# lasgroup/Model-based-policy-optimizers

Hardware: AMD Instinct MI355X
Metric: model-rollout transitions/sec + SAC updates/sec, Pendulum 5-ens h=5 (higher is better)
Workload: dtype f32

## Files before the change

### include/mbpo_hip.h

```cpp
#ifndef MBPO_HIP_H
#define MBPO_HIP_H

#include <stdint.h>

#ifdef __cplusplus
extern "C" {
#endif

#define MBPO_OK 0
#define MBPO_ERR_ARG (-1)
#define MBPO_ERR_UNSUPPORTED (-2)
#define MBPO_ERR_LAUNCH (-3)

#define MBPO_MAX_LAYERS 8

#define MBPO_ACT_SWISH 0
#define MBPO_ACT_RELU 1
#define MBPO_ACT_TANH 2

typedef struct mbpo_mlp_desc {
  const float *params;
  int64_t net_stride;
  int32_t n_nets;
  int32_t n_layers;
// ... 118 lines not shown
int mbpo_replay_sample_mixed(const float *data, int64_t max_size, int32_t row_len, const int32_t *state, const float *real_data,
                             int64_t real_max_size, int32_t real_row_len, const int32_t *real_state, uint64_t seed, uint64_t offset,
                             uint64_t real_offset, const uint64_t *rng_dev, int64_t n, int32_t minibatch, int32_t n_real,
                             int32_t *idx_out, float *out, void *stream);

int mbpo_philox_permutation(uint64_t seed, uint64_t offset, const uint64_t *rng_dev, int64_t n, int32_t *perm,
                            uint32_t *workspace, void *stream);

int64_t mbpo_running_stats_workspace_floats(int32_t x_dim);
int mbpo_running_stats_reduce(const float *rows, int64_t n_rows, int32_t row_len, int32_t col_off, int32_t x_dim,
                              const float *stats, float *sums, float *workspace, int32_t pass, void *stream);
int mbpo_running_stats_apply(float *stats, const float *sums, int32_t x_dim, float std_min, float std_max, void *stream);
int mbpo_running_stats_update(const float *rows, int64_t n_rows, int32_t row_len, int32_t col_off, int32_t x_dim, float *stats,
                              float *sums, float *workspace, float std_min, float std_max, void *stream);

int mbpo_gae_scan(const float *truncation, const float *termination, const float *rewards, const float *values,
                  const float *bootstrap, float *vs, float *advantages, int64_t B, int32_t T, float gamma,
                  float lam, int32_t time_major, void *stream);
int mbpo_lambda_return_scan(const float *rewards, const float *next_values, float *returns, int64_t B, int32_t T,
                            float gamma, float lam, int32_t time_major, void *stream);
int mbpo_gae_scan_discounts(const float *truncation, const float *termination, const float *rewards, const float *values,
                            const float *bootstrap, const float *discounts, float *vs, float *advantages, int64_t B,
                            int32_t T, float lam, int32_t time_major, void *stream);

typedef struct mbpo_sac_desc {
  int32_t x_dim, u_dim;
  int32_t policy_layers;
  int32_t policy_dims[MBPO_MAX_LAYERS + 1];
  int32_t q_layers;
  int32_t q_dims[MBPO_MAX_LAYERS + 1];
// ... 209 lines not shown
```

### model-based-policy-optimizers_amd/csrc/knobs.hpp

```cpp
#pragma once

#define MBPO_KNOB_TABLE(X)                                                                                                          \
  X(SAC_LEAN, "MBPO_SAC_LEAN", 1, false, "0: the generic k_sac_fwd_bwd also where k_sac_lean applies")                             \
  X(SAC_LAYERED, "MBPO_SAC_LAYERED", 0, false, "1: force SAC's layer-by-layer path (tests)")                                        \
  X(SAC_SPLIT, "MBPO_SAC_SPLIT", -1, false, "0/1: two / three workgroups per SAC tile; -1: by network shape")                       \
  X(SAC_JVP, "MBPO_SAC_JVP", -1, false, "0: no forward-mode dQ/da in SAC's actor role; -1: where the shapes allow it")              \
        \
  X(SAC_THIN, "MBPO_SAC_THIN", 1, true, "0: SAC's thin first / last layers go through the MFMA runners too")                        \
  X(PPO_LEAN, "MBPO_PPO_LEAN", 1, false, "0: the generic PPO kernels also where k_ppo_lean / k_ppo_vg_lean apply")                  \
  X(PPO_LAYERED, "MBPO_PPO_LAYERED", 0, false, "1: force PPO's layer-by-layer path (tests)")                                        \
  X(PPO_SP2, "MBPO_PPO_SP2", -1, false, "0: never the 512-thread two-per-CU k_ppo_fwd_bwd; -1: by shape and tile count")            \
  X(PPO_VALUES_GAE, "MBPO_PPO_VALUES_GAE", -1, false, "0: separate values / GAE / moments launches; -1: fused where it fits")       \
  X(ENS_LEAN, "MBPO_ENS_LEAN", 1, false, "0: the generic k_ensemble_forward also where k_ens_fwd_lean applies")                     \
  X(ROLLOUT_LEAN, "MBPO_ROLLOUT_LEAN", 1, false, "0 generic 64-wide rollout kernel, 1 k_rollout_lean, 2 / 3 lean with two tiles in flight forced on / off") \
  X(ROLLOUT_PIPE, "MBPO_ROLLOUT_PIPE", -1, false, "0/1: two tiles in flight per k_rollout_lean workgroup off / on; -1: by tile count") \
  X(LAYERED_T2_MIN, "MBPO_LAYERED_T2_MIN", 4096, false, "64x64-tile count from which the layered GEMM keeps 64x64 tiles (below: 32x32)") \
  X(LAYERED_GROUP, "MBPO_LAYERED_GROUP", 1, false, "0: every layered GEMM its own launch instead of one per dependency level")      \
  X(PERM_BUCKETS, "MBPO_PERM_BUCKETS", 1, false, "0: philox_permutation without the bucket pre-sort")                               \
  X(BPTT_ZSTORE_MAX_MB, "MBPO_BPTT_ZSTORE_MAX_MB", 16384, false, "largest BPTT member pre-activation store; above it the backward sweep recomputes") \
  X(ICEM_UPDATE, nullptr, -1, false, "override only: 0 the global-memory k_icem_update, 1 k_icem_update_lds where it fits")         \
  X(BPTT_ZSTORE, nullptr, -1, false, "override only: 0 no BPTT pre-activation store (recompute)")

enum KnobId {
#define MBPO_KNOB_ID_(id, env, dflt, reread, meaning) KNOB_##id,
  MBPO_KNOB_TABLE(MBPO_KNOB_ID_)
#undef MBPO_KNOB_ID_
  KNOB_COUNT
};

long long mbpo_knob(KnobId id);
int mbpo_knob_override(KnobId id);
int mbpo_knob_set_override(KnobId id, int mode);
```

### model-based-policy-optimizers_amd/csrc/replay.hip

```cpp
#include "common.hpp"
#include <stdlib.h>

struct ReplayPos {
  int pos, roll, head;
};

__device__ __forceinline__ ReplayPos replay_plan(const int *state, long long max_size, long long n) {
  ReplayPos p;
  long long pos = state[0];
  long long roll = max_size - pos - n;
  if (roll > 0) roll = 0;
  p.roll = (int)roll;
  p.pos = (int)(pos + roll);
  p.head = (int)(((long long)state[2] - roll) % max_size);
  return p;
}

__global__ void __launch_bounds__(256) k_replay_insert(float *data, long long max_size, int D, const int *state,
                                                        const float *rows, long long n_rows) {
  const ReplayPos p = replay_plan(state, max_size, n_rows);
  const long long s0 = ((long long)p.pos + p.head) % max_size;
  const long long n1 = (max_size - s0) < n_rows ? (max_size - s0) : n_rows;
  const long long e1 = n1 * D, total = n_rows * D;
  float *dst1 = data + s0 * D;
  const long long gtid = (long long)blockIdx.x * blockDim.x + threadIdx.x, gsz = (long long)gridDim.x * blockDim.x;
  const bool vec = ((e1 | total) & 3) == 0 && ((((unsigned long long)dst1) | ((unsigned long long)data) | ((unsigned long long)rows)) & 15ull) == 0;
  if (vec) {
    const f32x4 *src = reinterpret_cast<const f32x4 *>(rows);
    f32x4 *d1 = reinterpret_cast<f32x4 *>(dst1), *d2 = reinterpret_cast<f32x4 *>(data);
    const long long q1 = e1 >> 2, qt = total >> 2;
    for (long long i = gtid; i < qt; i += gsz) {
      const f32x4 v = src[i];
      if (i < q1) d1[i] = v;
      else d2[i - q1] = v;
    }
  } else {
    for (long long i = gtid; i < total; i += gsz) {
      const float v = rows[i];
      if (i < e1) dst1[i] = v;
      else data[i - e1] = v;
    }
  }
}

__global__ void k_replay_advance(int *state, long long max_size, long long n_rows) {
  if (threadIdx.x == 0 && blockIdx.x == 0) {
    const ReplayPos p = replay_plan(state, max_size, n_rows);
    long long newpos = ((long long)p.pos + n_rows) % (max_size + 1);
    long long sp = (long long)state[1] + p.roll;
    state[0] = (int)newpos;
    state[1] = (int)(sp > 0 ? sp : 0);
    state[2] = p.head;
    state[3] = (int)((unsigned)state[3] + (unsigned)n_rows);
  }
}

extern "C" int mbpo_replay_insert(float *data, int64_t max_size, int32_t row_len, int32_t *state, const float *rows,
                                  int64_t n_rows, void *stream) {
  MBPO_REQUIRE(data && state, MBPO_ERR_ARG, "replay_insert: null pointer");
  MBPO_REQUIRE(max_size > 0 && max_size < (1LL << 31) - 1 && row_len > 0, MBPO_ERR_ARG, "replay_insert: bad max_size/row_len");
  MBPO_REQUIRE(n_rows >= 0 && n_rows <= max_size, MBPO_ERR_ARG,
               "replay_insert: %lld rows do not fit a buffer of %lld rows", (long long)n_rows, (long long)max_size);
  if (n_rows == 0) return MBPO_OK;
  MBPO_REQUIRE(rows, MBPO_ERR_ARG, "replay_insert: null rows");
  long long total = n_rows * row_len;
  int grid = (int)((total + 255) / 256 < 2048 ? (total + 255) / 256 : 2048);
  hipStream_t st = (hipStream_t)stream;
  hipLaunchKernelGGL(k_replay_insert, dim3(grid), dim3(256), 0, st, data, (long long)max_size, row_len, state, rows,
                     (long long)n_rows);
  hipLaunchKernelGGL(k_replay_advance, dim3(1), dim3(64), 0, st, state, (long long)max_size, (long long)n_rows);
  MBPO_CHECK_LAUNCH("replay_insert");
  return MBPO_OK;
}

static int gather_rows_per_block(int row_len) {
  const int pieces = (row_len & 3) == 0 ? row_len >> 2 : row_len;
  int rb = (2048 + pieces - 1) / pieces;
  return rb < 1 ? 1 : (rb > 256 ? 256 : rb);
}

template <bool SAMPLE>
__global__ void __launch_bounds__(256) k_replay_gather(const float *data, long long max_size, int D, const int *state,
                                                        const int *idx, unsigned long long seed, unsigned long long offset,
                                                        const unsigned long long *rng_dev, long long n, int *idx_out, float *out, int RB) {
  __shared__ long long s_phys[256];
  if (SAMPLE) {
    const RngKey rk = rng_resolve(seed, offset, rng_dev);
    seed = rk.seed;
    offset = rk.offset;
  }
  const int head = state[2];
  const int lo = state[1], hi = state[0];
  const int tid = threadIdx.x;
  const bool vec = (D & 3) == 0 && ((((unsigned long long)data) | ((unsigned long long)out)) & 15ull) == 0;
  for (long long row0 = (long long)blockIdx.x * RB; row0 < n; row0 += (long long)gridDim.x * RB) {
    const long long j = row0 + tid;
    if (tid < RB && j < n) {
      long long li;
      if (SAMPLE) {
        li = philox_randint(seed, offset, MBPO_STREAM_REPLAY, (unsigned long long)j, lo, hi);
        if (idx_out) idx_out[j] = (int)li;
      } else {
        li = idx[j];
      }
      long long w = li % max_size;
      if (w < 0) w += max_size;
      s_phys[tid] = (w + head) % max_size;
    }
    __syncthreads();
    const int rows_here = (int)((n - row0) < RB ? (n - row0) : RB);
// ... 3 lines not shown
      f32x4 *dst = reinterpret_cast<f32x4 *>(out) + row0 * D4;
      for (int e = tid; e < total; e += 256) {
        const int r = e / D4, c = e - r * D4;
        dst[e] = src[s_phys[r] * D4 + c];
      }
    } else {
      const int total = rows_here * D;
      float *dst = out + row0 * D;
      for (int e = tid; e < total; e += 256) {
        const int r = e / D, c = e - r * D;
        dst[e] = data[s_phys[r] * D + c];
      }
    }
    __syncthreads();
  }
}

extern "C" int mbpo_replay_gather(const float *data, int64_t max_size, int32_t row_len, const int32_t *state,
                                  const int32_t *idx, int64_t n, float *out, void *stream) {
  MBPO_REQUIRE(data && state, MBPO_ERR_ARG, "replay_gather: null pointer");
  MBPO_REQUIRE(max_size > 0 && row_len > 0 && n >= 0, MBPO_ERR_ARG, "replay_gather: bad sizes");
  if (n == 0) return MBPO_OK;
  MBPO_REQUIRE(idx && out, MBPO_ERR_ARG, "replay_gather: null idx/out");
  const int RB = gather_rows_per_block(row_len);
  int grid = (int)((n + RB - 1) / RB < 4096 ? (n + RB - 1) / RB : 4096);
  hipLaunchKernelGGL(k_replay_gather<false>, dim3(grid), dim3(256), 0, (hipStream_t)stream, data, (long long)max_size, row_len,
                     state, idx, 0ull, 0ull, (const unsigned long long *)nullptr, (long long)n, (int *)nullptr, out, RB);
  MBPO_CHECK_LAUNCH("replay_gather");
  return MBPO_OK;
}
// ... 99 lines not shown
                     (unsigned long long)offset, (unsigned long long)real_offset, (const unsigned long long *)rng_dev, (long long)n,
                     minibatch, n_real, idx_out, out, RB);
  MBPO_CHECK_LAUNCH("replay_sample_mixed");
  return MBPO_OK;
}

#define STATS_WGS 512

__device__ __forceinline__ float wave_sum(float v) {
#pragma unroll
  for (int o = 32; o > 0; o >>= 1) v += __shfl_down(v, o, 64);
  return v;
}

template <int PASS>
__global__ void __launch_bounds__(256) k_stats_partial(const float *rows, long long n_rows, int D, int col_off, int X,
                                                        const float *stats, const float *sums, float *partial) {
  const int tid = threadIdx.x;
  const float *mean = stats + 1;
  const int rows_per_pass = 256 / X;
  const int c = tid % X, r0 = tid / X;
  float acc = 0.f;
  if (r0 < rows_per_pass) {
    const float m = mean[c];
    float upd = 0.f;
    if (PASS == 1) upd = sums[1 + c] / (stats[0] + sums[0]);
    for (long long r = (long long)blockIdx.x * rows_per_pass + r0; r < n_rows; r += (long long)gridDim.x * rows_per_pass) {
      float d = rows[r * D + col_off + c] - m;
      acc += (PASS == 0) ? d : d * (d - upd);
    }
  }
  __shared__ float s_all[256];
  s_all[tid] = acc;
  __syncthreads();
  if (tid < X) {
    float a = 0.f;
    for (int t = tid; t < rows_per_pass * X; t += X) a += s_all[t];
    partial[(long long)blockIdx.x * X + tid] = a;
  }
}

__device__ __forceinline__ float stats_column_sums(const float *partial, int n_parts, int X, float *s_sl) {
  const int tid = threadIdx.x;
  const int nsl = 256 / X, c = tid % X, sl = tid / X;
  float acc = 0.f;
  if (sl < nsl) {
    int g = sl;
    for (; g + 7 * nsl < n_parts; g += 8 * nsl) {
      float v[8];
#pragma unroll
      for (int k = 0; k < 8; ++k) v[k] = partial[(long long)(g + k * nsl) * X + c];
#pragma unroll
      for (int k = 0; k < 8; ++k) acc += v[k];
    }
// ... 57 lines not shown
    float s = sqrtf(fmaxf(nsv, 0.f) / count);
    sd[c] = fminf(fmaxf(s, std_min), std_max);
  }
  __syncthreads();
  if (c == 0) stats[0] = count;
}

extern "C" int mbpo_running_stats_apply(float *stats, const float *sums, int32_t x_dim, float std_min, float std_max, void *stream) {
  MBPO_REQUIRE(stats && sums, MBPO_ERR_ARG, "running_stats_apply: null pointer");
  MBPO_REQUIRE(x_dim > 0 && x_dim <= 128, MBPO_ERR_ARG, "running_stats_apply: x_dim out of range");
  hipLaunchKernelGGL(k_stats_apply, dim3(1), dim3(128), 0, (hipStream_t)stream, stats, sums, x_dim, std_min, std_max);
  MBPO_CHECK_LAUNCH("running_stats_apply");
  return MBPO_OK;
}

__global__ void __launch_bounds__(256) k_stats_pass1_fused(const float *rows, long long n_rows, int D, int col_off, int X,
                                                           const float *stats, const float *partial0, int n_parts0, float *sums,
                                                           float *partial1) {
  __shared__ float s_all[256];
  __shared__ float s_sum0[128];
  const int tid = threadIdx.x;
  const float tot = stats_column_sums(partial0, n_parts0, X, s_all);
  if (tid < X) {
    s_sum0[tid] = tot;
    if (blockIdx.x == 0) sums[1 + tid] = tot;
  }
  if (blockIdx.x == 0 && tid == 0) sums[0] = (float)n_rows;
  __syncthreads();
  const float *mean = stats + 1;
  const int rows_per_pass = 256 / X;
  const int c = tid % X, r0 = tid / X;
  float acc = 0.f;
  if (r0 < rows_per_pass) {
    const float m = mean[c];
    const float upd = s_sum0[c] / (stats[0] + (float)n_rows);
    for (long long r = (long long)blockIdx.x * rows_per_pass + r0; r < n_rows; r += (long long)gridDim.x * rows_per_pass) {
      float d = rows[r * D + col_off + c] - m;
      acc += d * (d - upd);
    }
  }
  s_all[tid] = acc;
  __syncthreads();
  if (tid < X) {
    float a = 0.f;
    for (int t = tid; t < rows_per_pass * X; t += X) a += s_all[t];
    partial1[(long long)blockIdx.x * X + tid] = a;
  }
}

__global__ void __launch_bounds__(256) k_stats_sums1_apply(const float *partial1, int n_parts, int X, float *sums, float *stats,
                                                           float std_min, float std_max) {
  __shared__ float s_sl[256];
  const int c = threadIdx.x;
  const float a = stats_column_sums(partial1, n_parts, X, s_sl);
  const float count = stats[0] + sums[0];
  if (c < X) {
    sums[1 + X + c] = a;
    if (count > 0.f) {
      float *mean = stats + 1, *sv = stats + 1 + X, *sd = stats + 1 + 2 * X;
      mean[c] = mean[c] + sums[1 + c] / count;
      float nsv = sv[c] + a;
      sv[c] = nsv;
      float s = sqrtf(fmaxf(nsv, 0.f) / count);
      sd[c] = fminf(fmaxf(s, std_min), std_max);
    }
  }
  __syncthreads();
  if (c == 0) stats[0] = count;
}

extern "C" int mbpo_running_stats_update(const float *rows, int64_t n_rows, int32_t row_len, int32_t col_off, int32_t x_dim,
                                         float *stats, float *sums, float *workspace, float std_min, float std_max, void *stream) {
  MBPO_REQUIRE(stats && sums && workspace, MBPO_ERR_ARG, "running_stats_update: null pointer");
  MBPO_REQUIRE(x_dim > 0 && x_dim <= 128 && row_len > 0 && col_off >= 0 && col_off + x_dim <= row_len, MBPO_ERR_ARG,
               "running_stats_update: bad column range (x_dim must be <= 128)");
  MBPO_REQUIRE(n_rows >= 0 && (n_rows == 0 || rows), MBPO_ERR_ARG, "running_stats_update: bad rows");
  hipStream_t st = (hipStream_t)stream;
  int rows_per_pass = 256 / x_dim;
  long long want = (n_rows + rows_per_pass - 1) / rows_per_pass;
  int grid = (int)(want < 1 ? 1 : (want < STATS_WGS ? want : STATS_WGS));
  float *partial1 = workspace + (long long)STATS_WGS * x_dim;
  hipLaunchKernelGGL(k_stats_partial<0>, dim3(grid), dim3(256), 0, st, rows, (long long)n_rows, row_len, col_off, x_dim,
                     (const float *)stats, (const float *)sums, workspace);
  hipLaunchKernelGGL(k_stats_pass1_fused, dim3(grid), dim3(256), 0, st, rows, (long long)n_rows, row_len, col_off, x_dim,
                     (const float *)stats, (const float *)workspace, grid, sums, partial1);
  hipLaunchKernelGGL(k_stats_sums1_apply, dim3(1), dim3(256), 0, st, (const float *)partial1, grid, x_dim, sums, stats, std_min, std_max);
  MBPO_CHECK_LAUNCH("running_stats_update");
  return MBPO_OK;
}

__global__ void __launch_bounds__(256) k_perm_keys(unsigned long long seed, unsigned long long offset, const unsigned long long *rng_dev,
                                                    long long n, unsigned int *keys) {
  const RngKey rk = rng_resolve(seed, offset, rng_dev);
  const long long i = (long long)blockIdx.x * 256 + threadIdx.x;
  if (i >= n) return;
  Philox4 p = philox4x32_10((uint32_t)i, (uint32_t)((unsigned long long)i >> 32), MBPO_STREAM_PERM ^ (uint32_t)(rk.offset >> 32) * 0x9E3779B9u,
                            (uint32_t)rk.offset, (uint32_t)rk.seed, (uint32_t)(rk.seed >> 32));
  keys[i] = p.v[0];
}

__global__ void __launch_bounds__(256) k_perm_rank(const unsigned int *keys, long long n, int *perm) {
  __shared__ unsigned int s_k[1024];
// ... 140 lines not shown
```

### model-based-policy-optimizers_amd/mbpo/_hip.py

```python
from __future__ import annotations

import ctypes as C
import os
from pathlib import Path
from typing import Optional, Sequence

import torch

MBPO_MAX_LAYERS = 8
ACT_IDS = {"swish": 0, "silu": 0, "relu": 1, "tanh": 2}

SYS_PENDULUM, SYS_ENSEMBLE = 0, 1
SYS_GENERIC = 100
ENS_MEAN, ENS_TS1, ENS_TSINF = 0, 1, 2
STREAM_POLICY_NOISE, STREAM_MODEL_NOISE, STREAM_MEMBER = 1, 2, 3
REWARD_PENDULUM, REWARD_QUADRATIC, REWARD_LEARNED = 0, 1, 2

_LIB_PATH = Path(__file__).resolve().parent / "_lib" / "libmbpo_hip.so"


class P2pDesc(C.Structure):
    _fields_ = [("world", C.c_int32), ("rank", C.c_int32), ("n_max", C.c_int64), ("regions", C.c_void_p * 16)]


# ... 178 lines not shown
    _bind_optional(lib)
    _lib = lib
    return lib


def _bind_optional(lib: C.CDLL) -> None:
    i32, i64, u64, f32, vp = C.c_int32, C.c_int64, C.c_uint64, C.c_float, C.c_void_p
    sigs = {
        "mbpo_replay_insert": [vp, i64, i32, vp, vp, i64, vp],
        "mbpo_replay_gather": [vp, i64, i32, vp, vp, i64, vp, vp],
        "mbpo_replay_sample": [vp, i64, i32, vp, u64, u64, vp, i64, vp, vp, vp],
        "mbpo_replay_sample_mixed": [vp, i64, i32, vp, vp, i64, i32, vp, u64, u64, u64, vp, i64, i32, i32, vp, vp, vp],
        "mbpo_running_stats_reduce": [vp, i64, i32, i32, i32, vp, vp, vp, i32, vp],
        "mbpo_running_stats_apply": [vp, vp, i32, f32, f32, vp],
        "mbpo_running_stats_update": [vp, i64, i32, i32, i32, vp, vp, vp, f32, f32, vp],
        "mbpo_gae_scan": [vp, vp, vp, vp, vp, vp, vp, i64, i32, f32, f32, i32, vp],
        "mbpo_gae_scan_discounts": [vp, vp, vp, vp, vp, vp, vp, vp, i64, i32, f32, i32, vp],
        "mbpo_lambda_return_scan": [vp, vp, vp, i64, i32, f32, f32, i32, vp],
        "mbpo_critic_grads": [vp, i32, i32, vp, i32, vp, i32, vp, vp, i64, vp, vp, vp, vp, vp, vp],
        "mbpo_adamw_step": [vp, vp, vp, vp, vp, i64, f32, f32, f32, i32, vp, f32, vp, vp, vp],
        "mbpo_rng_advance": [vp, u64, vp],
        "mbpo_soft_update": [vp, vp, vp, i64, f32, vp],
        "mbpo_philox_permutation": [u64, u64, vp, i64, vp, vp, vp],
    }
    for name, argtypes in sigs.items():
        fn = getattr(lib, name, None)
        if fn is not None:
            fn.restype = C.c_int
            fn.argtypes = argtypes
    for name in ("mbpo_sac_grads", "mbpo_sac_grad_norms", "mbpo_sac_apply", "mbpo_sac_step", "mbpo_sac_finalize"):
# ... 160 lines not shown
```

### model-based-policy-optimizers_amd/mbpo/ops.py

```python
from __future__ import annotations

import ctypes as C
import os
from dataclasses import dataclass
from typing import Optional, Sequence

import torch

from . import _hip
from ._hip import check, current_stream_ptr, load, mlp_desc, ptr, require_device_tensor as _req


@dataclass
class MlpSpec:
    dims: Sequence[int]
    activation: str = "swish"
    n_nets: int = 1

    @property
    def n_params(self) -> int:
        d = list(self.dims)
        return sum(d[i] * d[i + 1] + d[i + 1] for i in range(len(d) - 1))

    @property
# ... 562 lines not shown
        if workspace.numel() < stats_workspace_floats(x_dim):
            raise ValueError(f"workspace must hold {stats_workspace_floats(x_dim)} floats, got {workspace.numel()}")
        check(lib.mbpo_running_stats_update(rows.data_ptr(), rows.shape[0], rows.shape[1], col_off, x_dim, stats.data_ptr(),
                                            sums.data_ptr(), workspace.data_ptr(), std_min, std_max, current_stream_ptr()),
              "mbpo_running_stats_update")
        return
    sums = running_stats_reduce(rows, col_off, x_dim, stats, 0, sums=sums, workspace=workspace)
    if all_reduce is not None:
        all_reduce(sums)
    running_stats_reduce(rows, col_off, x_dim, stats, 1, sums=sums, workspace=workspace)
    if all_reduce is not None:
        all_reduce(sums[1 + x_dim:])
    running_stats_apply(stats, sums, x_dim, std_min, std_max)


def running_stats_apply(stats: torch.Tensor, sums: torch.Tensor, x_dim: int, std_min: float = 1e-6, std_max: float = 1e6) -> None:
    lib = load()
    _req(stats, "stats"); _req(sums, "sums")
    check(lib.mbpo_running_stats_apply(stats.data_ptr(), sums.data_ptr(), x_dim, std_min, std_max, current_stream_ptr()),
          "mbpo_running_stats_apply")


def gae_scan(truncation, termination, rewards, values, bootstrap, gamma, lam: float, time_major: bool = False):
    lib = load()
    for t, nm in ((truncation, "truncation"), (termination, "termination"), (rewards, "rewards"), (values, "values"),
                  (bootstrap, "bootstrap")):
        _req(t, nm)
    B, T = (values.shape[1], values.shape[0]) if time_major else (values.shape[0], values.shape[1])
    if bootstrap.shape != (B,):
        raise ValueError("bootstrap must be [B]")
# ... 826 lines not shown
```

### model-based-policy-optimizers_amd/mbpo/optimizers/policy_optimizers/sac/sac.py

```python
from __future__ import annotations

import dataclasses
import math
import os
import time
from dataclasses import dataclass
from typing import Any, Callable, Dict, List, Optional, Sequence, Tuple

import torch

from mbpo import _hip, ops
from mbpo.optimizers.policy_optimizers.brax_utils.base import LearnerState, State, rehome_state
from mbpo.parallel import DataParallel
from mbpo.replay import ReplayBufferState, UniformSamplingQueue
from mbpo.systems.brax_wrapper import BraxWrapper
from mbpo.systems.ensemble_system import lecun_uniform_flat
from mbpo.systems.time_adaptive import check_trainer
from mbpo.types import Transition
from mbpo.utils import keys as K

Metrics = Dict[str, Any]

SITE_ROLLOUT, SITE_SAMPLE, SITE_SAMPLE_REAL, SITE_SGD = 1, 2, 3, 16

# ... 281 lines not shown
        if self.eval_env is self.env:
            self.eval_env = environment
        self.env = environment

    def _training_state(self, env_steps: int) -> TrainingState:
        u = self.updater
        return TrainingState(policy_optimizer_state=(u.adam_m[:u.P], u.adam_v[:u.P]), policy_params=u.policy_params,
                             q_optimizer_state=(u.adam_m[u.P:u.P + 2 * u.Q], u.adam_v[u.P:u.P + 2 * u.Q]),
                             q_params=u.q_params, target_q_params=u.target_q, gradient_steps=u.step_count,
                             env_steps=env_steps, alpha_optimizer_state=(u.adam_m[-1:], u.adam_v[-1:]),
                             alpha_params=u.log_alpha, normalizer_params=RunningStatisticsState(self._stats_vec, self.x_dim))

    def rekey(self, key: int) -> None:
        ops.set_rng(self._rng, K.PRNGKey(key), 0)

    def get_experience(self, normalizer_params: RunningStatisticsState, policy_params: torch.Tensor, env_state: State,
                       buffer_state: ReplayBufferState, key: Optional[int] = None):
        if key is not None:
            self.rekey(key)
        nm, ns = self._norm(normalizer_params)
        spec = self.env.system.rollout_spec(env_state.system_params, self.device)
        sp_out: list = []
        rows = ops.model_rollout(policy_params=policy_params, policy_spec=self.policy_spec, x_dim=self.x_dim, u_dim=self.u_dim,
                                 obs=env_state.obs, first_obs=env_state.info['first_obs'], steps=env_state.info['steps'],
                                 done=env_state.done, n_steps=self.num_env_steps_between_updates,
                                 episode_length=self.episode_length, action_repeat=self.action_repeat, norm_mean=nm,
                                 norm_std=ns, seed=0, offset=SITE_ROLLOUT << 32, rng_dev=self._rng,
                                 out=self._rollout_rows, system_params_out=sp_out, **spec, **self._start_buffer())
        if sp_out:
            env_state = env_state.replace(system_params=sp_out[-1])
        ops.running_stats_update(rows, 0, self.x_dim, normalizer_params.vec, all_reduce=self._all_reduce,
                                 sums=self._stats_sums, workspace=self._stats_ws)
        buffer_state = self.replay_buffer.insert_rows(buffer_state, rows)
        return normalizer_params, env_state, buffer_state

    def _start_buffer(self) -> dict:
        if not self.resample_starts:
            return {}
        real = self.env.sample_buffer_state
        return dict(start_rows=real.data, start_state=real.state)

    def sgd_step(self, transitions_rows: torch.Tensor, normalizer_params: RunningStatisticsState, key: Optional[int] = None,
                 g: int = 0, defer_clip_check: bool = False) -> None:
        if key is not None:
            self.rekey(key)
        nm, ns = self._norm(normalizer_params)
        self.updater.sgd_step(transitions_rows, nm, ns, seed=0, offset=(SITE_SGD + g) << 32, rng_dev=self._rng,
                              defer_clip_check=defer_clip_check)

    def training_step(self, training_state: TrainingState, env_state: State, buffer_state: ReplayBufferState,
                      key: Optional[int] = None):
        if key is not None:
            self.rekey(key)
        normalizer_params, env_state, buffer_state = self.get_experience(
            training_state.normalizer_params, training_state.policy_params, env_state, buffer_state)
        training_state = training_state.replace(
            env_steps=training_state.env_steps + self.env_steps_per_actor_step * self.num_env_steps_between_updates)
        if self.n_real == 0:
            buffer_state, rows = self.replay_buffer.sample_rows(buffer_state, out=self._batch_rows, seed=0,
                                                                offset=SITE_SAMPLE << 32, rng_dev=self._rng)
        else:
            buffer_state, rows = self.replay_buffer.sample_rows_mixed(
                buffer_state, self.env.sample_buffer, self.env.sample_buffer_state, self.n_real, self.batch_size,
                out=self._batch_rows, seed=0, offset=SITE_SAMPLE << 32, real_offset=SITE_SAMPLE_REAL << 32, rng_dev=self._rng)
        B = self.batch_size
        for g in range(self.grad_updates_per_step):
            self.sgd_step(rows[g * B:(g + 1) * B], normalizer_params, g=g, defer_clip_check=True)
        self.updater.finalize(rng_dev=self._rng)
        return training_state, env_state, buffer_state

    def prefill_replay_buffer(self, training_state: TrainingState, env_state: State, buffer_state: ReplayBufferState, key: int,
                              num_steps: Optional[int] = None):
        key, new_key = K.split(key)
        self.rekey(key)
        for _ in range(self.num_prefill_actor_steps if num_steps is None else num_steps):
            _, env_state, buffer_state = self.get_experience(training_state.normalizer_params, training_state.policy_params,
# ... 213 lines not shown
```

### model-based-policy-optimizers_amd/mbpo/replay.py

```python
from __future__ import annotations

import dataclasses
from dataclasses import dataclass
from typing import Optional, Tuple

import torch

from . import ops
from .types import Transition, flatten, row_layout, unflatten
from .utils import keys as K


@dataclass
class ReplayBufferState:
    data: torch.Tensor
    state: torch.Tensor
    key: int
    insert_position: int = 0
    sample_position: int = 0
    head: int = 0
    sample_count: int = 0

    def replace(self, **kw):
        return dataclasses.replace(self, **kw)
# ... 42 lines not shown
        pos = bs.insert_position + roll
        return bs.replace(insert_position=(pos + n) % (mx + 1), sample_position=max(0, bs.sample_position + roll),
                          head=(bs.head - roll) % mx)

    def sample_rows(self, bs: ReplayBufferState, n: Optional[int] = None, out: Optional[torch.Tensor] = None,
                    rng_dev: Optional[torch.Tensor] = None, seed: Optional[int] = None, offset: int = 0
                    ) -> Tuple[ReplayBufferState, torch.Tensor]:
        n = self.sample_batch_size if n is None else n
        if self.size(bs) <= 0:
            raise ValueError("cannot sample from an empty replay buffer")
        key, sample_key = K.split(bs.key)
        rows = ops.replay_sample(bs.data, bs.state, n, seed=sample_key if seed is None else seed, offset=offset, out=out,
                                 rng_dev=rng_dev)
        return bs.replace(key=key, sample_count=bs.sample_count + 1), rows

    def check_mixable(self, real_queue: "UniformSamplingQueue") -> None:
        if (real_queue.x_dim, real_queue.u_dim) != (self.x_dim, self.u_dim):
            raise ValueError(f"cannot mix rows of a buffer with (x_dim, u_dim) = ({real_queue.x_dim}, {real_queue.u_dim}) into one with "
                             f"({self.x_dim}, {self.u_dim})")
        if real_queue.ppo_extras or self.ppo_extras:
            raise ValueError("cannot mix rows that carry PPO policy extras (log_prob, raw_action)")
        if real_queue.row_len > self.row_len:
            raise ValueError(f"real rows of {real_queue.row_len} floats do not fit rows of {self.row_len}")

    def sample_rows_mixed(self, bs: ReplayBufferState, real_queue: "UniformSamplingQueue", real_bs: ReplayBufferState, n_real: int,
                          minibatch: int, n: Optional[int] = None, out: Optional[torch.Tensor] = None,
                          rng_dev: Optional[torch.Tensor] = None, seed: Optional[int] = None, offset: int = 0,
                          real_offset: int = 0, idx_out: Optional[torch.Tensor] = None
                          ) -> Tuple[ReplayBufferState, torch.Tensor]:
        n = self.sample_batch_size if n is None else n
# ... 15 lines not shown
```

Baseline: 19.43 million.

## Fuse running-stats update, replay insert and sample into three launches

Adds an experience_tail entry point that merges the running-statistics reduction, the replay-buffer insert, the state advance and the minibatch sample into three kernels instead of six separate launches. Work is split across workgroups within each kernel, so the stats pass and the insert share a launch, and the second stats pass shares one with the gather. SAC's get_experience routes through it when observations are normalized with no all-reduce and no real-data mixing. This is meant to cut launch overhead in the small-batch SAC loop, at the cost of more complex kernels with SGPR-pinning asm and branching over workgroup ranges.

```diff
diff --git a/include/mbpo_hip.h b/include/mbpo_hip.h
--- a/include/mbpo_hip.h
+++ b/include/mbpo_hip.h
@@ -156,6 +156,11 @@
 int mbpo_running_stats_update(const float *rows, int64_t n_rows, int32_t row_len, int32_t col_off, int32_t x_dim, float *stats,
                               float *sums, float *workspace, float std_min, float std_max, void *stream);
 
+int mbpo_experience_tail(const float *rows, int64_t n_rows, int32_t row_len, int32_t col_off, int32_t x_dim, float *stats,
+                         float *sums, float *stats_scratch, float std_min, float std_max, float *data, int64_t max_size,
+                         int32_t *state, uint64_t seed, uint64_t offset, const uint64_t *rng_dev, int64_t n_sample,
+                         int32_t *idx_out, float *out, void *stream);
+
 int mbpo_gae_scan(const float *truncation, const float *termination, const float *rewards, const float *values,
                   const float *bootstrap, float *vs, float *advantages, int64_t B, int32_t T, float gamma,
                   float lam, int32_t time_major, void *stream);
diff --git a/model-based-policy-optimizers_amd/csrc/knobs.hpp b/model-based-policy-optimizers_amd/csrc/knobs.hpp
--- a/model-based-policy-optimizers_amd/csrc/knobs.hpp
+++ b/model-based-policy-optimizers_amd/csrc/knobs.hpp
@@ -17,6 +17,8 @@
   X(LAYERED_T2_MIN, "MBPO_LAYERED_T2_MIN", 4096, false, "64x64-tile count from which the layered GEMM keeps 64x64 tiles (below: 32x32)") \
   X(LAYERED_GROUP, "MBPO_LAYERED_GROUP", 1, false, "0: every layered GEMM its own launch instead of one per dependency level")      \
   X(PERM_BUCKETS, "MBPO_PERM_BUCKETS", 1, false, "0: philox_permutation without the bucket pre-sort")                               \
+   \
+  X(EXPERIENCE_TAIL, "MBPO_EXPERIENCE_TAIL", 1, false, "0: mbpo_experience_tail issues the six stand-alone launches instead of its three") \
   X(BPTT_ZSTORE_MAX_MB, "MBPO_BPTT_ZSTORE_MAX_MB", 16384, false, "largest BPTT member pre-activation store; above it the backward sweep recomputes") \
   X(ICEM_UPDATE, nullptr, -1, false, "override only: 0 the global-memory k_icem_update, 1 k_icem_update_lds where it fits")         \
   X(BPTT_ZSTORE, nullptr, -1, false, "override only: 0 no BPTT pre-activation store (recompute)")
diff --git a/model-based-policy-optimizers_amd/csrc/replay.hip b/model-based-policy-optimizers_amd/csrc/replay.hip
--- a/model-based-policy-optimizers_amd/csrc/replay.hip
+++ b/model-based-policy-optimizers_amd/csrc/replay.hip
@@ -5,25 +5,43 @@
   int pos, roll, head;
 };
 
-__device__ __forceinline__ ReplayPos replay_plan(const int *state, long long max_size, long long n) {
+__device__ __forceinline__ ReplayPos replay_plan(int insert_position, int head, long long max_size, long long n) {
   ReplayPos p;
-  long long pos = state[0];
+  long long pos = insert_position;
   long long roll = max_size - pos - n;
   if (roll > 0) roll = 0;
   p.roll = (int)roll;
   p.pos = (int)(pos + roll);
-  p.head = (int)(((long long)state[2] - roll) % max_size);
+  p.head = (int)(((long long)head - roll) % max_size);
   return p;
 }
 
-__global__ void __launch_bounds__(256) k_replay_insert(float *data, long long max_size, int D, const int *state,
-                                                        const float *rows, long long n_rows) {
+__device__ __forceinline__ ReplayPos replay_plan(const int *state, long long max_size, long long n) {
+  return replay_plan(state[0], state[2], max_size, n);
+}
+
+struct ReplayWords {
+  int hi, lo, head;
+};
+
+__device__ __forceinline__ ReplayWords replay_advanced(int insert_position, int sample_position, int head, long long max_size,
+                                                       long long n) {
+  const ReplayPos p = replay_plan(insert_position, head, max_size, n);
+  ReplayWords a;
+  a.hi = (int)(((long long)p.pos + n) % (max_size + 1));
+  const long long sp = (long long)sample_position + p.roll;
+  a.lo = (int)(sp > 0 ? sp : 0);
+  a.head = p.head;
+  return a;
+}
+
+__device__ __forceinline__ void replay_insert_body(float *data, long long max_size, int D, const int *state, const float *rows,
+                                                   long long n_rows, long long gtid, long long gsz) {
   const ReplayPos p = replay_plan(state, max_size, n_rows);
   const long long s0 = ((long long)p.pos + p.head) % max_size;
   const long long n1 = (max_size - s0) < n_rows ? (max_size - s0) : n_rows;
   const long long e1 = n1 * D, total = n_rows * D;
   float *dst1 = data + s0 * D;
-  const long long gtid = (long long)blockIdx.x * blockDim.x + threadIdx.x, gsz = (long long)gridDim.x * blockDim.x;
   const bool vec = ((e1 | total) & 3) == 0 && ((((unsigned long long)dst1) | ((unsigned long long)data) | ((unsigned long long)rows)) & 15ull) == 0;
   if (vec) {
     const f32x4 *src = reinterpret_cast<const f32x4 *>(rows);
@@ -43,15 +61,23 @@
   }
 }
 
+__global__ void __launch_bounds__(256) k_replay_insert(float *data, long long max_size, int D, const int *state,
+                                                        const float *rows, long long n_rows) {
+  replay_insert_body(data, max_size, D, state, rows, n_rows, (long long)blockIdx.x * blockDim.x + threadIdx.x,
+                     (long long)gridDim.x * blockDim.x);
+}
+
+__device__ __forceinline__ void replay_advance_store(int *state, const ReplayWords &a, int total_before, long long n_rows) {
+  state[0] = a.hi;
+  state[1] = a.lo;
+  state[2] = a.head;
+  state[3] = (int)((unsigned)total_before + (unsigned)n_rows);
+}
+
 __global__ void k_replay_advance(int *state, long long max_size, long long n_rows) {
   if (threadIdx.x == 0 && blockIdx.x == 0) {
-    const ReplayPos p = replay_plan(state, max_size, n_rows);
-    long long newpos = ((long long)p.pos + n_rows) % (max_size + 1);
-    long long sp = (long long)state[1] + p.roll;
-    state[0] = (int)newpos;
-    state[1] = (int)(sp > 0 ? sp : 0);
-    state[2] = p.head;
-    state[3] = (int)((unsigned)state[3] + (unsigned)n_rows);
+    const int s0 = state[0], s1 = state[1], s2 = state[2], total = state[3];
+    replay_advance_store(state, replay_advanced(s0, s1, s2, max_size, n_rows), total, n_rows);
   }
 }
 
@@ -80,20 +106,20 @@
 }
 
 template <bool SAMPLE>
-__global__ void __launch_bounds__(256) k_replay_gather(const float *data, long long max_size, int D, const int *state,
-                                                        const int *idx, unsigned long long seed, unsigned long long offset,
-                                                        const unsigned long long *rng_dev, long long n, int *idx_out, float *out, int RB) {
-  __shared__ long long s_phys[256];
+__device__ __forceinline__ void replay_gather_body(const float *data, long long max_size, int D, const ReplayWords w, const int *idx,
+                                                   unsigned long long seed, unsigned long long offset,
+                                                   const unsigned long long *rng_dev, long long n, int *idx_out, float *out, int RB,
+                                                   int bid, int nblk, long long *s_phys) {
   if (SAMPLE) {
     const RngKey rk = rng_resolve(seed, offset, rng_dev);
     seed = rk.seed;
     offset = rk.offset;
   }
-  const int head = state[2];
-  const int lo = state[1], hi = state[0];
+  const int head = w.head;
+  const int lo = w.lo, hi = w.hi;
   const int tid = threadIdx.x;
   const bool vec = (D & 3) == 0 && ((((unsigned long long)data) | ((unsigned long long)out)) & 15ull) == 0;
-  for (long long row0 = (long long)blockIdx.x * RB; row0 < n; row0 += (long long)gridDim.x * RB) {
+  for (long long row0 = (long long)bid * RB; row0 < n; row0 += (long long)nblk * RB) {
     const long long j = row0 + tid;
     if (tid < RB && j < n) {
       long long li;
@@ -127,6 +153,19 @@
     }
     __syncthreads();
   }
+}
+
+template <bool SAMPLE>
+__global__ void __launch_bounds__(256) k_replay_gather(const float *data, long long max_size, int D, const int *state,
+                                                        const int *idx, unsigned long long seed, unsigned long long offset,
+                                                        const unsigned long long *rng_dev, long long n, int *idx_out, float *out, int RB) {
+  __shared__ long long s_phys[256];
+  ReplayWords w;
+  w.head = state[2];
+  w.lo = state[1];
+  w.hi = state[0];
+  replay_gather_body<SAMPLE>(data, max_size, D, w, idx, seed, offset, rng_dev, n, idx_out, out, RB, (int)blockIdx.x, (int)gridDim.x,
+                             s_phys);
 }
 
 extern "C" int mbpo_replay_gather(const float *data, int64_t max_size, int32_t row_len, const int32_t *state,
@@ -256,8 +295,8 @@
 }
 
 template <int PASS>
-__global__ void __launch_bounds__(256) k_stats_partial(const float *rows, long long n_rows, int D, int col_off, int X,
-                                                        const float *stats, const float *sums, float *partial) {
+__device__ __forceinline__ void stats_partial_body(const float *rows, long long n_rows, int D, int col_off, int X, const float *stats,
+                                                   const float *sums, float *partial, int bid, int nblk, float *s_all) {
   const int tid = threadIdx.x;
   const float *mean = stats + 1;
   const int rows_per_pass = 256 / X;
@@ -267,19 +306,25 @@
     const float m = mean[c];
     float upd = 0.f;
     if (PASS == 1) upd = sums[1 + c] / (stats[0] + sums[0]);
-    for (long long r = (long long)blockIdx.x * rows_per_pass + r0; r < n_rows; r += (long long)gridDim.x * rows_per_pass) {
+    for (long long r = (long long)bid * rows_per_pass + r0; r < n_rows; r += (long long)nblk * rows_per_pass) {
       float d = rows[r * D + col_off + c] - m;
       acc += (PASS == 0) ? d : d * (d - upd);
     }
   }
-  __shared__ float s_all[256];
   s_all[tid] = acc;
   __syncthreads();
   if (tid < X) {
     float a = 0.f;
     for (int t = tid; t < rows_per_pass * X; t += X) a += s_all[t];
-    partial[(long long)blockIdx.x * X + tid] = a;
-  }
+    partial[(long long)bid * X + tid] = a;
+  }
+}
+
+template <int PASS>
+__global__ void __launch_bounds__(256) k_stats_partial(const float *rows, long long n_rows, int D, int col_off, int X,
+                                                        const float *stats, const float *sums, float *partial) {
+  __shared__ float s_all[256];
+  stats_partial_body<PASS>(rows, n_rows, D, col_off, X, stats, sums, partial, (int)blockIdx.x, (int)gridDim.x, s_all);
 }
 
 __device__ __forceinline__ float stats_column_sums(const float *partial, int n_parts, int X, float *s_sl) {
@@ -367,18 +412,16 @@
   return MBPO_OK;
 }
 
-__global__ void __launch_bounds__(256) k_stats_pass1_fused(const float *rows, long long n_rows, int D, int col_off, int X,
-                                                           const float *stats, const float *partial0, int n_parts0, float *sums,
-                                                           float *partial1) {
-  __shared__ float s_all[256];
-  __shared__ float s_sum0[128];
+__device__ __forceinline__ void stats_pass1_fused_body(const float *rows, long long n_rows, int D, int col_off, int X,
+                                                       const float *stats, const float *partial0, int n_parts0, float *sums,
+                                                       float *partial1, int bid, int nblk, float *s_all, float *s_sum0) {
   const int tid = threadIdx.x;
   const float tot = stats_column_sums(partial0, n_parts0, X, s_all);
   if (tid < X) {
     s_sum0[tid] = tot;
-    if (blockIdx.x == 0) sums[1 + tid] = tot;
-  }
-  if (blockIdx.x == 0 && tid == 0) sums[0] = (float)n_rows;
+    if (bid == 0) sums[1 + tid] = tot;
+  }
+  if (bid == 0 && tid == 0) sums[0] = (float)n_rows;
   __syncthreads();
   const float *mean = stats + 1;
   const int rows_per_pass = 256 / X;
@@ -387,7 +430,7 @@
   if (r0 < rows_per_pass) {
     const float m = mean[c];
     const float upd = s_sum0[c] / (stats[0] + (float)n_rows);
-    for (long long r = (long long)blockIdx.x * rows_per_pass + r0; r < n_rows; r += (long long)gridDim.x * rows_per_pass) {
+    for (long long r = (long long)bid * rows_per_pass + r0; r < n_rows; r += (long long)nblk * rows_per_pass) {
       float d = rows[r * D + col_off + c] - m;
       acc += d * (d - upd);
     }
@@ -397,13 +440,21 @@
   if (tid < X) {
     float a = 0.f;
     for (int t = tid; t < rows_per_pass * X; t += X) a += s_all[t];
-    partial1[(long long)blockIdx.x * X + tid] = a;
-  }
-}
-
-__global__ void __launch_bounds__(256) k_stats_sums1_apply(const float *partial1, int n_parts, int X, float *sums, float *stats,
-                                                           float std_min, float std_max) {
-  __shared__ float s_sl[256];
+    partial1[(long long)bid * X + tid] = a;
+  }
+}
+
+__global__ void __launch_bounds__(256) k_stats_pass1_fused(const float *rows, long long n_rows, int D, int col_off, int X,
+                                                           const float *stats, const float *partial0, int n_parts0, float *sums,
+                                                           float *partial1) {
+  __shared__ float s_all[256];
+  __shared__ float s_sum0[128];
+  stats_pass1_fused_body(rows, n_rows, D, col_off, X, stats, partial0, n_parts0, sums, partial1, (int)blockIdx.x, (int)gridDim.x, s_all,
+                         s_sum0);
+}
+
+__device__ __forceinline__ void stats_sums1_apply_body(const float *partial1, int n_parts, int X, float *sums, float *stats,
+                                                       float std_min, float std_max, float *s_sl) {
   const int c = threadIdx.x;
   const float a = stats_column_sums(partial1, n_parts, X, s_sl);
   const float count = stats[0] + sums[0];
@@ -420,6 +471,12 @@
   }
   __syncthreads();
   if (c == 0) stats[0] = count;
+}
+
+__global__ void __launch_bounds__(256) k_stats_sums1_apply(const float *partial1, int n_parts, int X, float *sums, float *stats,
+                                                           float std_min, float std_max) {
+  __shared__ float s_sl[256];
+  stats_sums1_apply_body(partial1, n_parts, X, sums, stats, std_min, std_max, s_sl);
 }
 
 extern "C" int mbpo_running_stats_update(const float *rows, int64_t n_rows, int32_t row_len, int32_t col_off, int32_t x_dim,
@@ -439,6 +496,145 @@
                      (const float *)stats, (const float *)workspace, grid, sums, partial1);
   hipLaunchKernelGGL(k_stats_sums1_apply, dim3(1), dim3(256), 0, st, (const float *)partial1, grid, x_dim, sums, stats, std_min, std_max);
   MBPO_CHECK_LAUNCH("running_stats_update");
+  return MBPO_OK;
+}
+
+struct TailArgs {
+  const float *rows;
+  float *stats, *sums, *partial0, *partial1, *data, *out;
+  int *state, *idx_out;
+  const unsigned long long *rng_dev;
+  long long n_rows, max_size, n_sample;
+  unsigned long long seed, offset;
+  int D, col_off, X, g_stats, g_insert, g_sample, RB;
+  float std_min, std_max;
+};
+
+typedef __attribute__((address_space(1))) float TailGF;
+typedef __attribute__((address_space(1))) int TailGI;
+typedef __attribute__((address_space(1))) unsigned long long TailGU;
+
+__global__ void __launch_bounds__(256) k_tail_pass0_insert(TailArgs A) {
+  __shared__ float s_all[256];
+  TailGF *g_rows = (TailGF *)A.rows, *g_stats_v = (TailGF *)A.stats, *g_partial0 = (TailGF *)A.partial0, *g_data = (TailGF *)A.data;
+  TailGI *g_state = (TailGI *)A.state;
+  long long n_rows = A.n_rows, max_size = A.max_size;
+  int D = A.D, col_off = A.col_off, X = A.X, g_stats = A.g_stats, g_insert = A.g_insert;
+  asm("" : "+s"(g_rows), "+s"(g_stats_v), "+s"(g_partial0), "+s"(g_data), "+s"(g_state), "+s"(n_rows), "+s"(max_size), "+s"(D),
+               "+s"(col_off), "+s"(X), "+s"(g_stats), "+s"(g_insert));
+  const float *rows = (const float *)g_rows;
+  const int bid = (int)blockIdx.x;
+  if (bid < g_stats) {
+    stats_partial_body<0>(rows, n_rows, D, col_off, X, (const float *)g_stats_v, (const float *)nullptr, (float *)g_partial0, bid,
+                          g_stats, s_all);
+  } else {
+    replay_insert_body((float *)g_data, max_size, D, (const int *)g_state, rows, n_rows, (long long)(bid - g_stats) * 256 + threadIdx.x,
+                       (long long)g_insert * 256);
+  }
+}
+
+__global__ void __launch_bounds__(256) k_tail_pass1_sample(TailArgs A) {
+  __shared__ float s_all[256];
+  __shared__ float s_sum0[128];
+  __shared__ long long s_phys[256];
+  TailGF *g_rows = (TailGF *)A.rows, *g_stats_v = (TailGF *)A.stats, *g_partial0 = (TailGF *)A.partial0,
+         *g_partial1 = (TailGF *)A.partial1, *g_sums = (TailGF *)A.sums, *g_data = (TailGF *)A.data, *g_out = (TailGF *)A.out;
+  TailGI *g_state = (TailGI *)A.state, *g_idx_out = (TailGI *)A.idx_out;
+  TailGU *g_rng = (TailGU *)A.rng_dev;
+  long long n_rows = A.n_rows, max_size = A.max_size, n_sample = A.n_sample;
+  unsigned long long seed = A.seed, offset = A.offset;
+  int D = A.D, col_off = A.col_off, X = A.X, g_stats = A.g_stats, g_sample = A.g_sample, RB = A.RB;
+  asm("" : "+s"(g_rows), "+s"(g_stats_v), "+s"(g_partial0), "+s"(g_partial1), "+s"(g_sums), "+s"(g_data), "+s"(g_out), "+s"(g_state),
+               "+s"(g_idx_out), "+s"(g_rng), "+s"(n_rows), "+s"(max_size), "+s"(n_sample), "+s"(seed), "+s"(offset));
+  asm("" : "+s"(D), "+s"(col_off), "+s"(X), "+s"(g_stats), "+s"(g_sample), "+s"(RB));
+  const int bid = (int)blockIdx.x;
+  if (bid < g_stats) {
+    stats_pass1_fused_body((const float *)g_rows, n_rows, D, col_off, X, (const float *)g_stats_v, (const float *)g_partial0, g_stats,
+                           (float *)g_sums, (float *)g_partial1, bid, g_stats, s_all, s_sum0);
+  } else {
+    const int *state = (const int *)g_state;
+    const int s0 = state[0], s1 = state[1], s2 = state[2];
+    const RngKey rk = rng_resolve(seed, offset, (const unsigned long long *)g_rng);
+    const ReplayWords w = replay_advanced(s0, s1, s2, max_size, n_rows);
+    replay_gather_body<true>((const float *)g_data, max_size, D, w, (const int *)nullptr, rk.seed, rk.offset,
+                             (const unsigned long long *)nullptr, n_sample, (int *)g_idx_out, (float *)g_out, RB, bid - g_stats, g_sample,
+                             s_phys);
+  }
+}
+
+__global__ void __launch_bounds__(256) k_tail_apply_advance(TailArgs A) {
+  __shared__ float s_sl[256];
+  TailGF *g_partial1 = (TailGF *)A.partial1, *g_sums = (TailGF *)A.sums, *g_stats_v = (TailGF *)A.stats;
+  TailGI *g_state = (TailGI *)A.state;
+  long long n_rows = A.n_rows, max_size = A.max_size;
+  int X = A.X, g_stats = A.g_stats;
+  float std_min = A.std_min, std_max = A.std_max;
+  asm("" : "+s"(g_partial1), "+s"(g_sums), "+s"(g_stats_v), "+s"(g_state), "+s"(n_rows), "+s"(max_size), "+s"(X), "+s"(g_stats),
+               "+s"(std_min), "+s"(std_max));
+  int *state = (int *)g_state;
+  const int s0 = state[0], s1 = state[1], s2 = state[2], total = state[3];
+  stats_sums1_apply_body((const float *)g_partial1, g_stats, X, (float *)g_sums, (float *)g_stats_v, std_min, std_max, s_sl);
+  if (threadIdx.x == 0) replay_advance_store(state, replay_advanced(s0, s1, s2, max_size, n_rows), total, n_rows);
+}
+
+extern "C" int mbpo_debug_set_experience_tail(int mode) { return mbpo_knob_set_override(KNOB_EXPERIENCE_TAIL, mode); }
+
+extern "C" int mbpo_experience_tail(const float *rows, int64_t n_rows, int32_t row_len, int32_t col_off, int32_t x_dim, float *stats,
+                                    float *sums, float *stats_scratch, float std_min, float std_max, float *data, int64_t max_size,
+                                    int32_t *state, uint64_t seed, uint64_t offset, const uint64_t *rng_dev, int64_t n_sample,
+                                    int32_t *idx_out, float *out, void *stream) {
+  MBPO_REQUIRE(stats && sums && stats_scratch && data && state, MBPO_ERR_ARG, "experience_tail: null pointer");
+  MBPO_REQUIRE(x_dim > 0 && x_dim <= 128 && row_len > 0 && col_off >= 0 && col_off + x_dim <= row_len, MBPO_ERR_ARG,
+               "experience_tail: bad column range (x_dim must be <= 128)");
+  MBPO_REQUIRE(max_size > 0 && max_size < (1LL << 31) - 1, MBPO_ERR_ARG, "experience_tail: bad max_size");
+  MBPO_REQUIRE(n_rows >= 0 && n_rows <= max_size, MBPO_ERR_ARG, "experience_tail: %lld rows do not fit a buffer of %lld rows",
+               (long long)n_rows, (long long)max_size);
+  MBPO_REQUIRE(n_rows == 0 || rows, MBPO_ERR_ARG, "experience_tail: null rows");
+  MBPO_REQUIRE(n_sample >= 0 && (n_sample == 0 || out), MBPO_ERR_ARG, "experience_tail: bad n_sample / null out");
+  if (mbpo_knob(KNOB_EXPERIENCE_TAIL) == 0 || n_rows == 0) {
+    int rc = mbpo_running_stats_update(rows, n_rows, row_len, col_off, x_dim, stats, sums, stats_scratch, std_min, std_max, stream);
+    if (rc != MBPO_OK) return rc;
+    rc = mbpo_replay_insert(data, max_size, row_len, state, rows, n_rows, stream);
+    if (rc != MBPO_OK) return rc;
+    return mbpo_replay_sample(data, max_size, row_len, state, seed, offset, rng_dev, n_sample, idx_out, out, stream);
+  }
+  hipStream_t st = (hipStream_t)stream;
+  const int rows_per_pass = 256 / x_dim;
+  const long long want = (n_rows + rows_per_pass - 1) / rows_per_pass;
+  const int g_stats = (int)(want < STATS_WGS ? want : STATS_WGS);
+  const long long total = n_rows * row_len;
+  const int g_insert = (int)((total + 255) / 256 < 2048 ? (total + 255) / 256 : 2048);
+  const int RB = gather_rows_per_block(row_len);
+  const int g_sample = (int)((n_sample + RB - 1) / RB < 4096 ? (n_sample + RB - 1) / RB : 4096);
+  TailArgs A;
+  A.rows = rows;
+  A.stats = stats;
+  A.sums = sums;
+  A.partial0 = stats_scratch;
+  A.partial1 = stats_scratch + (long long)STATS_WGS * x_dim;
+  A.data = data;
+  A.out = out;
+  A.state = state;
+  A.idx_out = idx_out;
+  A.rng_dev = (const unsigned long long *)rng_dev;
+  A.n_rows = n_rows;
+  A.max_size = max_size;
+  A.n_sample = n_sample;
+  A.seed = seed;
+  A.offset = offset;
+  A.D = row_len;
+  A.col_off = col_off;
+  A.X = x_dim;
+  A.g_stats = g_stats;
+  A.g_insert = g_insert;
+  A.g_sample = g_sample;
+  A.RB = RB;
+  A.std_min = std_min;
+  A.std_max = std_max;
+  hipLaunchKernelGGL(k_tail_pass0_insert, dim3(g_stats + g_insert), dim3(256), 0, st, A);
+  hipLaunchKernelGGL(k_tail_pass1_sample, dim3(g_stats + g_sample), dim3(256), 0, st, A);
+  hipLaunchKernelGGL(k_tail_apply_advance, dim3(1), dim3(256), 0, st, A);
+  MBPO_CHECK_LAUNCH("experience_tail");
   return MBPO_OK;
 }
 
diff --git a/model-based-policy-optimizers_amd/mbpo/_hip.py b/model-based-policy-optimizers_amd/mbpo/_hip.py
--- a/model-based-policy-optimizers_amd/mbpo/_hip.py
+++ b/model-based-policy-optimizers_amd/mbpo/_hip.py
@@ -216,6 +216,8 @@
         "mbpo_running_stats_reduce": [vp, i64, i32, i32, i32, vp, vp, vp, i32, vp],
         "mbpo_running_stats_apply": [vp, vp, i32, f32, f32, vp],
         "mbpo_running_stats_update": [vp, i64, i32, i32, i32, vp, vp, vp, f32, f32, vp],
+        "mbpo_experience_tail": [vp, i64, i32, i32, i32, vp, vp, vp, f32, f32, vp, i64, vp, u64, u64, vp, i64, vp, vp, vp],
+        "mbpo_debug_set_experience_tail": [i32],
         "mbpo_gae_scan": [vp, vp, vp, vp, vp, vp, vp, i64, i32, f32, f32, i32, vp],
         "mbpo_gae_scan_discounts": [vp, vp, vp, vp, vp, vp, vp, vp, i64, i32, f32, i32, vp],
         "mbpo_lambda_return_scan": [vp, vp, vp, i64, i32, f32, f32, i32, vp],
diff --git a/model-based-policy-optimizers_amd/mbpo/ops.py b/model-based-policy-optimizers_amd/mbpo/ops.py
--- a/model-based-policy-optimizers_amd/mbpo/ops.py
+++ b/model-based-policy-optimizers_amd/mbpo/ops.py
@@ -600,6 +600,37 @@
     running_stats_apply(stats, sums, x_dim, std_min, std_max)
 
 
+def experience_tail(rows: torch.Tensor, col_off: int, x_dim: int, stats: torch.Tensor, sums: torch.Tensor, workspace: torch.Tensor,
+                    data: torch.Tensor, state: torch.Tensor, n_sample: int = 0, seed: int = 0, offset: int = 0,
+                    out: Optional[torch.Tensor] = None, rng_dev: Optional[torch.Tensor] = None,
+                    idx_out: Optional[torch.Tensor] = None, std_min: float = 1e-6, std_max: float = 1e6) -> Optional[torch.Tensor]:
+    lib = load()
+    _req(rows, "rows"); _req(stats, "stats"); _req(sums, "sums"); _req(workspace, "workspace"); _req(data, "data")
+    _req(state, "state", torch.int32)
+    if rows.dim() != 2 or data.dim() != 2 or rows.shape[1] != data.shape[1]:
+        raise ValueError(f"rows must be [n, row_len] with data's row_len, got {tuple(rows.shape)} and {tuple(data.shape)}")
+    if stats.numel() != 1 + 3 * x_dim or sums.numel() < 1 + 2 * x_dim:
+        raise ValueError("stats must be [1 + 3*x_dim] and sums hold 1 + 2*x_dim floats")
+    if workspace.numel() < stats_workspace_floats(x_dim):
+        raise ValueError(f"workspace must hold {stats_workspace_floats(x_dim)} floats, got {workspace.numel()}")
+    if n_sample > 0:
+        if out is None:
+            out = torch.empty((n_sample, data.shape[1]), device=data.device, dtype=torch.float32)
+        else:
+            _req(out, "out")
+            if out.numel() < n_sample * data.shape[1]:
+                raise ValueError(f"out must hold {n_sample} rows of {data.shape[1]} floats")
+    if idx_out is not None:
+        _req(idx_out, "idx_out", torch.int32)
+        if idx_out.numel() != n_sample:
+            raise ValueError(f"idx_out must have {n_sample} entries")
+    check(lib.mbpo_experience_tail(rows.data_ptr(), rows.shape[0], rows.shape[1], col_off, x_dim, stats.data_ptr(), sums.data_ptr(),
+                                   workspace.data_ptr(), std_min, std_max, data.data_ptr(), data.shape[0], state.data_ptr(), seed,
+                                   offset, rng_ptr(rng_dev), n_sample, ptr(idx_out), ptr(out) if n_sample > 0 else None,
+                                   current_stream_ptr()), "mbpo_experience_tail")
+    return out if n_sample > 0 else None
+
+
 def running_stats_apply(stats: torch.Tensor, sums: torch.Tensor, x_dim: int, std_min: float = 1e-6, std_max: float = 1e6) -> None:
     lib = load()
     _req(stats, "stats"); _req(sums, "sums")
diff --git a/model-based-policy-optimizers_amd/mbpo/optimizers/policy_optimizers/sac/sac.py b/model-based-policy-optimizers_amd/mbpo/optimizers/policy_optimizers/sac/sac.py
--- a/model-based-policy-optimizers_amd/mbpo/optimizers/policy_optimizers/sac/sac.py
+++ b/model-based-policy-optimizers_amd/mbpo/optimizers/policy_optimizers/sac/sac.py
@@ -319,8 +319,11 @@
     def rekey(self, key: int) -> None:
         ops.set_rng(self._rng, K.PRNGKey(key), 0)
 
+    def _tail_eligible(self) -> bool:
+        return self.normalize_observations and self._all_reduce is None and self.n_real == 0
+
     def get_experience(self, normalizer_params: RunningStatisticsState, policy_params: torch.Tensor, env_state: State,
-                       buffer_state: ReplayBufferState, key: Optional[int] = None):
+                       buffer_state: ReplayBufferState, key: Optional[int] = None, sample: Optional[dict] = None):
         if key is not None:
             self.rekey(key)
         nm, ns = self._norm(normalizer_params)
@@ -334,9 +337,19 @@
                                  out=self._rollout_rows, system_params_out=sp_out, **spec, **self._start_buffer())
         if sp_out:
             env_state = env_state.replace(system_params=sp_out[-1])
-        ops.running_stats_update(rows, 0, self.x_dim, normalizer_params.vec, all_reduce=self._all_reduce,
-                                 sums=self._stats_sums, workspace=self._stats_ws)
-        buffer_state = self.replay_buffer.insert_rows(buffer_state, rows)
+        if self._tail_eligible():
+            req = sample or {}
+            buffer_state, sampled = self.replay_buffer.experience_tail(
+                buffer_state, rows, 0, self.x_dim, normalizer_params.vec, self._stats_sums, self._stats_ws,
+                n_sample=req["out"].shape[0] if sample else 0, out=req.get("out"), rng_dev=req.get("rng_dev"), seed=0,
+                offset=req.get("offset", 0))
+        else:
+            ops.running_stats_update(rows, 0, self.x_dim, normalizer_params.vec, all_reduce=self._all_reduce,
+                                     sums=self._stats_sums, workspace=self._stats_ws)
+            buffer_state = self.replay_buffer.insert_rows(buffer_state, rows)
+            sampled = None
+        if sample is not None:
+            return normalizer_params, env_state, buffer_state, sampled
         return normalizer_params, env_state, buffer_state
 
     def _start_buffer(self) -> dict:
@@ -357,14 +370,15 @@
                       key: Optional[int] = None):
         if key is not None:
             self.rekey(key)
-        normalizer_params, env_state, buffer_state = self.get_experience(
-            training_state.normalizer_params, training_state.policy_params, env_state, buffer_state)
+        normalizer_params, env_state, buffer_state, rows = self.get_experience(
+            training_state.normalizer_params, training_state.policy_params, env_state, buffer_state,
+            sample=dict(out=self._batch_rows, offset=SITE_SAMPLE << 32, rng_dev=self._rng))
         training_state = training_state.replace(
             env_steps=training_state.env_steps + self.env_steps_per_actor_step * self.num_env_steps_between_updates)
-        if self.n_real == 0:
+        if rows is None and self.n_real == 0:
             buffer_state, rows = self.replay_buffer.sample_rows(buffer_state, out=self._batch_rows, seed=0,
                                                                 offset=SITE_SAMPLE << 32, rng_dev=self._rng)
-        else:
+        elif rows is None:
             buffer_state, rows = self.replay_buffer.sample_rows_mixed(
                 buffer_state, self.env.sample_buffer, self.env.sample_buffer_state, self.n_real, self.batch_size,
                 out=self._batch_rows, seed=0, offset=SITE_SAMPLE << 32, real_offset=SITE_SAMPLE_REAL << 32, rng_dev=self._rng)
diff --git a/model-based-policy-optimizers_amd/mbpo/replay.py b/model-based-policy-optimizers_amd/mbpo/replay.py
--- a/model-based-policy-optimizers_amd/mbpo/replay.py
+++ b/model-based-policy-optimizers_amd/mbpo/replay.py
@@ -80,6 +80,24 @@
                                  rng_dev=rng_dev)
         return bs.replace(key=key, sample_count=bs.sample_count + 1), rows
 
+    def experience_tail(self, bs: ReplayBufferState, rows: torch.Tensor, col_off: int, x_dim: int, stats: torch.Tensor,
+                        sums: torch.Tensor, workspace: torch.Tensor, n_sample: int = 0, out: Optional[torch.Tensor] = None,
+                        rng_dev: Optional[torch.Tensor] = None, seed: Optional[int] = None, offset: int = 0
+                        ) -> Tuple[ReplayBufferState, Optional[torch.Tensor]]:
+        n = rows.shape[0]
+        if n > self.max_replay_size:
+            raise ValueError(f"cannot insert {n} rows into a buffer of {self.max_replay_size}")
+        after = self.insert_mirror(bs, n)
+        sample_key = 0
+        if n_sample > 0:
+            if self.size(after) <= 0:
+                raise ValueError("cannot sample from an empty replay buffer")
+            key, sample_key = K.split(bs.key)
+            after = after.replace(key=key, sample_count=bs.sample_count + 1)
+        sampled = ops.experience_tail(rows, col_off, x_dim, stats, sums, workspace, bs.data, bs.state, n_sample=n_sample,
+                                      seed=sample_key if seed is None else seed, offset=offset, out=out, rng_dev=rng_dev)
+        return after, sampled
+
     def check_mixable(self, real_queue: "UniformSamplingQueue") -> None:
         if (real_queue.x_dim, real_queue.u_dim) != (self.x_dim, self.u_dim):
             raise ValueError(f"cannot mix rows of a buffer with (x_dim, u_dim) = ({real_queue.x_dim}, {real_queue.u_dim}) into one with "
```

Result: no change. 19.59 million (median of 6 runs) (+0.8%).
